# FrozenWolf-Cyber/Indic-CL-ASR

Hardware: AMD Instinct MI355X
Metric: utterances/sec (15 s @16 kHz) Conformer-M RNNT-CTC+EWC train step (higher is better)
Workload: dtype bf16; 1 GPU; BASELINE configs[1]: Conformer-medium (d=256, 16L, H=640) hybrid RNNT-CTC + EWC, bs=32/GPU x 15 s, bf16 projections, freeze_encoder_till=12, 22x257 heads, fused_batch_size=4; global_batch=32, parallelism=dp1

## Files before the change

### include/indicasr.h

```cpp
#ifndef INDICASR_H
#define INDICASR_H

#include <stddef.h>
#include <stdint.h>

#ifdef __cplusplus
extern "C" {
#endif

typedef void* ia_stream_t;

enum ia_status {
    IA_OK = 0,
    IA_INVALID_VALUE = -1,
    IA_WORKSPACE_TOO_SMALL = -2,
    IA_LAUNCH_FAILED = -3,
    IA_UNSUPPORTED = -4,
};

const char* ia_version(void);

size_t ia_rnnt_workspace_bytes(int B, int T, int U1);
int ia_rnnt_loss(const float* logits, const int64_t* labels, const int64_t* act_lens, const int64_t* label_lens,
                 int B, int T, int U1, int V, int blank, float fastemit_lambda, float clamp,
// ... 89 lines not shown
                                int* counts, int* overflow, ia_stream_t stream);
size_t ia_greedy_decode_scratch_bytes(int B, int Hp, int Hj);
int ia_greedy_decode_cluster(int B, int Hp, int Hj);
int ia_greedy_rnnt_decode_bf16w_ex(const float* f_all, const int64_t* out_len, const float* EW, const void* Whh_bf16,
                                   const void* Wpred_bf16, const float* bpred, const void* Whead_bf16, const float* bhead, int B,
                                   int T, int Hp, int Hj, int V, int blank, int row_blank, int row_sos, int max_symbols, int* tokens,
                                   int cap, int* counts, int* overflow, int cluster, void* scratch, size_t scratch_bytes,
                                   ia_stream_t stream);

int ia_edit_distance_batch(const int32_t* a, const int64_t* a_off, const int32_t* b, const int64_t* b_off, int n, int64_t* out);

int ia_quantize_fp8_rows(const void* x, int is_f32, int ld, int64_t M, int K, void* q, int ldq, float* scale, ia_stream_t stream);
int ia_gemm_fp8(const void* Aq, int lda, const float* a_scale, const void* Wq, int ldw, const float* w_scale, int M, int N, int K,
                const float* bias, int act, float dropout_p, unsigned seed, float alpha, const float* R, int ldr, float* outF,
                int ldof, void* outH, int ldoh, ia_stream_t stream);
int ia_subsample_conv1(const float* feats, int B, int Fm, int Tm, int C, const float* w1, const float* b1, void* out,
                       ia_stream_t stream);
int ia_subsample_conv2(const void* in_cl, int B, int T1, int F1, int C, const void* w2r, const float* b2, int N, void* out,
                       ia_stream_t stream);
int ia_gemm_bf16_ln_supported(int N, int K);
int ia_gemm_bf16_ln(const void* A, int lda, const void* W, int ldw, int M, int N, int K, const float* bias, float dropout_p,
                    unsigned seed, float alpha, const float* R, int ldr, float* outF, int ldof, const float* ln_g,
                    const float* ln_b, float ln_eps, void* outH, int ldoh, ia_stream_t stream);
int ia_layernorm(const float* x, int ldx, int N, int d, const float* g1, const float* b1, float eps, float* outF,
                 int ldf, const float* g2, const float* b2, void* outH, int ldh, ia_stream_t stream);
int ia_glu_dwconv(const void* x2, const int64_t* lens, int B, int T, int d, int ksz, const float* w, const float* bias,
                  float* z, float* bn_sum, float* bn_sumsq, float* scratch, ia_stream_t stream);
int64_t ia_dwconv_scratch_elems(int B, int T, int d, int ksz);
int ia_colsum_bf16(const void* x, int M, int N, int ld, float* out, ia_stream_t stream);
int ia_dwconv_time(const float* x, int B, int T, int d, int ksz, const float* w, const float* bias, int flip, float* y,
                   ia_stream_t stream);
int ia_dwconv_time_wgrad(const float* x, const float* dy, int B, int T, int d, int ksz, float* dw, float* db,
                         float* scratch, ia_stream_t stream);
int ia_dwconv_glu_bwd(const float* dz, const void* c2, const int64_t* lens, int B, int T, int d, int ksz, const float* w, void* dc2,
                      ia_stream_t stream);
int ia_dwconv_glu_wgrad(const void* c2, const int64_t* lens, const float* dy, int B, int T, int d, int ksz, float* dw, float* db,
                        float* scratch, ia_stream_t stream);
int ia_bn_silu(const float* z, int64_t n_rows, int d, const float* bn_sum, const float* bn_sumsq, const float* gamma,
               const float* beta, float* running_mean, float* running_var, int64_t* num_batches_tracked,
               float momentum, float eps, int training, void* out, ia_stream_t stream);

int ia_gemm_bnsilu_supported(int K);
int ia_gemm_bnsilu_bf16(const float* z, int ldz, int64_t n_rows, const float* bn_sum, const float* bn_sumsq,
                        const float* gamma, const float* beta, float* running_mean, float* running_var,
                        int64_t* num_batches_tracked, float momentum, float eps, int training, const void* W, int ldw, int M,
                        int N, int K, const float* bias, float dropout_p, unsigned seed, float alpha, const float* R, int ldr,
// ... 230 lines not shown
```

### indic_cl_asr_amd/_lib.py

```python
import ctypes
import os
import subprocess

_HERE = os.path.dirname(os.path.abspath(__file__))
LIB_PATH = os.environ.get("IA_LIB_PATH") or os.path.join(_HERE, "libindicasr_hip.so")

IA_OK = 0
_STATUS = {-1: "IA_INVALID_VALUE", -2: "IA_WORKSPACE_TOO_SMALL", -3: "IA_LAUNCH_FAILED", -4: "IA_UNSUPPORTED"}

_c = ctypes
_vp, _i, _f, _sz = _c.c_void_p, _c.c_int, _c.c_float, _c.c_size_t
_i64 = _c.c_int64

class BlockParams(_c.Structure):
    _fields_ = ([(n, _c.c_void_p) for n in (
        "w_ff1a", "w_ff1b", "w_qkv", "w_pos", "w_out", "w_pw1", "w_pw2", "w_ff2a", "w_ff2b",
        "b_ff1a", "b_ff1b", "b_qkv", "b_out", "b_pw1", "b_pw2", "b_ff2a", "b_ff2b",
        "ln_ff1_g", "ln_ff1_b", "ln_att_g", "ln_att_b", "ln_conv_g", "ln_conv_b", "ln_ff2_g", "ln_ff2_b", "ln_out_g", "ln_out_b",
        "pos_u", "pos_v", "dw_w", "dw_b", "bn_g", "bn_b", "bn_rm", "bn_rv", "bn_nbt")]
        + [(n, _c.c_float) for n in ("ln_eps", "bn_eps", "bn_momentum", "p_drop", "p_ff", "p_att", "fc_factor")]
        + [(n, _c.c_int) for n in ("d", "d_ff", "n_heads", "ksz")]
        + [("pl_cached", _c.c_void_p), ("w_pw1_glu", _c.c_void_p), ("b_pw1_glu", _c.c_void_p)])


# ... 64 lines not shown
    "ia_quantize_mxfp8": (_i, [_vp, _i, _i, _i64, _i, _vp, _i, _vp, _i, _vp]),
    "ia_gemm_mxfp8": (_i, [_vp, _i, _vp, _i, _vp, _i, _vp, _i, _i, _i, _i, _vp, _i, _f, _c.c_uint, _f, _vp, _i, _vp, _i, _vp, _i, _vp]),
    "ia_cast_pad_bf16": (_i, [_vp, _i, _i64, _i, _vp, _i, _vp]),
    "ia_rnnt_lattice": (_i, [_vp, _vp, _i, _i, _i, _f, _i, _vp, _vp, _sz, _vp]),
    "ia_joint_backward_g": (_i, [_vp, _vp, _vp, _vp, _i, _i, _i, _i, _i, _i, _f, _vp, _f, _vp, _i, _i, _vp, _vp, _vp, _sz, _vp, _vp,
                                 _vp]),
    "ia_joint_backward_g_skip": (_i, [_vp, _vp, _vp, _vp, _i, _i, _i, _i, _i, _i, _f, _vp, _f, _vp, _i, _i, _vp, _vp, _vp, _sz, _i, _vp,
                                      _vp, _vp]),
    "ia_joint_backward_g_dbias_scratch_elems": (_i64, [_i]),
    "ia_joint_hidden_t": (_i, [_vp, _vp, _vp, _i, _i, _i, _i, _i, _i, _i, _f, _c.c_uint, _vp]),
    "ia_joint_hidden": (_i, [_vp, _vp, _vp, _i, _i, _i, _i, _i, _f, _c.c_uint, _vp]),
    "ia_joint_dh_reduce": (_i, [_vp, _vp, _vp, _vp, _vp, _vp, _vp, _i, _i, _i, _i, _f, _f, _c.c_uint, _vp, _vp]),
    "ia_joint_dh_reduce_scratch_bytes": (_sz, [_i, _i, _i, _i]),
    "ia_joint_dh_fused_supported": (_i, [_i, _i, _i]),
    "ia_joint_dh_k": (_i, []),
    "ia_joint_dh_fused": (_i, [_vp, _vp, _vp, _vp, _vp, _vp, _vp, _vp, _i, _i, _i, _i, _i, _f, _f, _c.c_uint, _vp, _vp]),
    "ia_joint_dh_fused_ex": (_i, [_vp, _vp, _vp, _vp, _vp, _vp, _vp, _vp, _vp, _vp, _i, _i, _i, _i, _i, _i, _f, _f, _c.c_uint, _vp, _vp]),
    "ia_joint_dh_fused_scratch_bytes": (_sz, [_i, _i, _i, _i]),
    "ia_joint_dw_fused_supported": (_i, [_i, _i, _i]),
    "ia_joint_dw_fused_scratch_elems": (_i64, [_i, _i, _i, _i, _i]),
    "ia_joint_dw_fused": (_i, [_vp, _vp, _vp, _vp, _i, _i, _i, _i, _i, _f, _c.c_uint, _vp, _vp, _vp]),
    "ia_gemm_bf16_ln_supported": (_i, [_i, _i]),
    "ia_gemm_bf16_ln": (_i, [_vp, _i, _vp, _i, _i, _i, _i, _vp, _f, _c.c_uint, _f, _vp, _i, _vp, _i, _vp, _vp, _f, _vp, _i, _vp]),
    "ia_joint_dw_fused_ex": (_i, [_vp, _vp, _vp, _vp, _vp, _i, _i, _i, _i, _i, _f, _c.c_uint, _vp, _vp, _vp]),
    "ia_gemm_bf16": (_i, [_vp, _i, _vp, _i, _i, _i, _i, _vp, _i, _f, _c.c_uint, _f, _vp, _i, _vp, _i, _vp, _i, _vp]),
    "ia_gemm_bf16_ex": (_i, [_vp, _i, _vp, _i, _i, _i, _i, _vp, _i, _f, _c.c_uint, _f, _vp, _i, _vp, _i, _vp, _i, _vp, _i, _vp, _i, _vp]),
    "ia_subsample_conv1": (_i, [_vp, _i, _i, _i, _i, _vp, _vp, _vp, _vp]),
    "ia_subsample_conv2": (_i, [_vp, _i, _i, _i, _i, _vp, _vp, _i, _vp, _vp]),
    "ia_layernorm": (_i, [_vp, _i, _i, _i, _vp, _vp, _f, _vp, _i, _vp, _vp, _vp, _i, _vp]),
    "ia_glu_dwconv": (_i, [_vp, _vp, _i, _i, _i, _i, _vp, _vp, _vp, _vp, _vp, _vp, _vp]),
    "ia_dwconv_scratch_elems": (_i64, [_i, _i, _i, _i]),
    "ia_colsum_bf16": (_i, [_vp, _i, _i, _i, _vp, _vp]),
    "ia_dwconv_time": (_i, [_vp, _i, _i, _i, _i, _vp, _vp, _i, _vp, _vp]),
    "ia_dwconv_time_wgrad": (_i, [_vp, _vp, _i, _i, _i, _i, _vp, _vp, _vp, _vp]),
    "ia_dwconv_glu_bwd": (_i, [_vp, _vp, _vp, _i, _i, _i, _i, _vp, _vp, _vp]),
    "ia_dwconv_glu_wgrad": (_i, [_vp, _vp, _vp, _i, _i, _i, _i, _vp, _vp, _vp, _vp]),
    "ia_bn_silu": (_i, [_vp, _i64, _i, _vp, _vp, _vp, _vp, _vp, _vp, _vp, _f, _f, _i, _vp, _vp]),
    "ia_gemm_bnsilu_supported": (_i, [_i]),
    "ia_gemm_bnsilu_bf16": (_i, [_vp, _i, _i64, _vp, _vp, _vp, _vp, _vp, _vp, _vp, _f, _f, _i, _vp, _i, _i, _i, _i, _vp, _f, _c.c_uint, _f,
                                 _vp, _i, _vp, _i, _vp, _i, _vp, _vp]),
    "ia_gemm_bnsilu_bf16_keep": (_i, [_vp, _i, _i64, _vp, _vp, _vp, _vp, _vp, _vp, _vp, _f, _f, _i, _vp, _i, _i, _i, _i, _vp, _f, _c.c_uint,
                                      _f, _vp, _i, _vp, _i, _vp, _i, _vp, _vp, _i, _vp]),
    "ia_glu_dwconv_fixed": (_i, [_vp, _vp, _i, _i, _i, _i, _vp, _vp, _vp, _vp, _vp]),
    "ia_dwconv_gated_fixed": (_i, [_vp, _vp, _i, _i, _i, _i, _vp, _vp, _vp, _vp, _vp]),
    "ia_attn_vt_elems": (_sz, [_i, _i, _i]),
    "ia_relpos_attention": (_i, [_vp, _vp, _vp, _vp, _vp, _i, _i, _i, _i, _f, _c.c_uint, _vp, _vp, _vp]),
# ... 103 lines not shown
```

### indic_cl_asr_amd/csrc/block_exec.hip

```cpp
#include <hip/hip_runtime.h>

#include <cstdint>
#include <cstdlib>

#include "indicasr.h"
#include "ia_common.h"

namespace {
inline size_t up256(size_t x) { return (x + 255) / 256 * 256; }
constexpr int PREFIX_ACC_LAYERS = 64;

struct PrefixWs {
    size_t y, h, qkv, pl, ctx, c2, z, sums, acc, c3, scr, total;
};

PrefixWs prefix_ws(int B, int T, int d, int d_ff, int ksz, int pos_rows) {
    const size_t N = (size_t)B * T;
    PrefixWs w;
    size_t o = 0;
    w.y = o;    o = up256(o + N * d * 2);
    w.h = o;    o = up256(o + N * d_ff * 2);
    w.qkv = o;  o = up256(o + N * 3 * d * 2);
    w.pl = o;   o = up256(o + (size_t)pos_rows * d * 2);
    w.ctx = o;  o = up256(o + N * d * 2);
// ... 39 lines not shown
    if (seg_begin < 0 || seg_end > 2 * n_layers || seg_begin >= seg_end) return IA_INVALID_VALUE;
    if (!layers || n_layers <= 0 || !x || !pos_emb || !lens || !workspace || B <= 0 || T <= 0) return IA_INVALID_VALUE;
    const ia_block_params& l0 = layers[0];
    const int d = l0.d, d_ff = l0.d_ff, H = l0.n_heads, dk = d / (H > 0 ? H : 1), ksz = l0.ksz;
    if (pos_rows < 2 * T - 1) return IA_INVALID_VALUE;
    const PrefixWs w = prefix_ws(B, T, d, d_ff, ksz, pos_rows);
    if (workspace_bytes < w.total) return IA_WORKSPACE_TOO_SMALL;
    if (H <= 0) return IA_INVALID_VALUE;
    if (!ia_relpos_attention_flash_supported(T, dk)) return IA_UNSUPPORTED;
    char* ws = (char*)workspace;
    void *y = ws + w.y, *h = ws + w.h, *qkv = ws + w.qkv, *pl = ws + w.pl, *ctx = ws + w.ctx, *c2 = ws + w.c2, *c3 = ws + w.c3;
    float *z = (float*)(ws + w.z), *sums = (float*)(ws + w.sums), *scr = (float*)(ws + w.scr);
    long long* acc = (long long*)(ws + w.acc);
    const int N = B * T;
    const char* ffn_env = getenv("IA_PREFIX_FFN");
    const bool ffn_fused = ia_ffn_fused_supported(d, d_ff) != 0 && !(ffn_env && ffn_env[0] == 'g');
    const char* bns_env = getenv("IA_PREFIX_BNSILU");
    const bool bnsilu_fused = ia_gemm_bnsilu_supported(d) != 0 && !(bns_env && bns_env[0] == 's');
    const bool bn_fixed = bnsilu_fused && !bn_synced && seg_begin == 0 && seg_end >= 2 * n_layers && n_layers <= PREFIX_ACC_LAYERS;
    if (bn_fixed && hipMemsetAsync(acc, 0, (size_t)n_layers * IA_BN_ACC_COPIES * 2 * d * sizeof(long long), (hipStream_t)stream) != hipSuccess)
        return IA_LAUNCH_FAILED;
    const char* glu_env = getenv("IA_PREFIX_GLU");
    const bool glu_in_gemm = d % 64 == 0 && !(glu_env && glu_env[0] == 'd');
    if (!ffn_fused && seg_begin == 0)
        IA_TRY(ia_layernorm(x, d, N, d, l0.ln_ff1_g, l0.ln_ff1_b, l0.ln_eps, nullptr, 0, nullptr, nullptr, y, d, stream));
    for (int li = seg_begin / 2; li < n_layers && 2 * li < seg_end; ++li) {
        const ia_block_params& L = layers[li];
        if (L.d != d || L.d_ff != d_ff || L.n_heads != H || L.ksz != ksz) return IA_INVALID_VALUE;
        const unsigned seed = seed_base + seed_stride * (unsigned)li;
        const float p = training ? L.p_drop : 0.f, pff = training ? L.p_ff : 0.f, patt = training ? L.p_att : 0.f;
        const bool first_half = 2 * li >= seg_begin, second_half = 2 * li + 1 < seg_end;
        if (first_half) {
        const char* tail_env = getenv("IA_FFN_TAIL");
        const bool qkv_tail = ffn_fused && !(tail_env && tail_env[0] == '0') && ia_ffn_fused_tail_supported(d, d_ff, 3 * d);
        if (qkv_tail) {
            IA_TRY(ia_ffn_fused_tail(x, N, d, d_ff, L.ln_ff1_g, L.ln_ff1_b, L.ln_eps, L.w_ff1a, L.b_ff1a, L.w_ff1b, L.b_ff1b, L.fc_factor,
                                     pff, seed + 1, p, seed + 2, L.ln_att_g, L.ln_att_b, nullptr, 1, L.w_qkv, L.b_qkv, qkv, 3 * d, stream));
        } else if (ffn_fused) {
            IA_TRY(ia_ffn_fused(x, N, d, d_ff, L.ln_ff1_g, L.ln_ff1_b, L.ln_eps, L.w_ff1a, L.b_ff1a, L.w_ff1b, L.b_ff1b, L.fc_factor,
                                pff, seed + 1, p, seed + 2, L.ln_att_g, L.ln_att_b, y, 1, stream));
        } else {
            IA_TRY(ia_gemm_bf16(y, d, L.w_ff1a, d, N, d_ff, d, L.b_ff1a, 1, pff, seed + 1, 1.f, nullptr, 0, nullptr, 0, h, d_ff, stream));
            IA_TRY(ia_gemm_bf16(h, d_ff, L.w_ff1b, d_ff, N, d, d_ff, L.b_ff1b, 0, p, seed + 2, L.fc_factor, x, d, x, d, nullptr, 0, stream));
        }
        if (!ffn_fused)
            IA_TRY(ia_layernorm(x, d, N, d, L.ln_att_g, L.ln_att_b, L.ln_eps, nullptr, 0, nullptr, nullptr, y, d, stream));
        if (!qkv_tail)
            IA_TRY(ia_gemm_bf16(y, d, L.w_qkv, d, N, 3 * d, d, L.b_qkv, 0, 0.f, 0, 1.f, nullptr, 0, nullptr, 0, qkv, 3 * d, stream));
        const void* plu = L.pl_cached;
        if (!plu) {
            IA_TRY(ia_gemm_bf16(pos_emb, d, L.w_pos, d, pos_rows, d, d, nullptr, 0, 0.f, 0, 1.f, nullptr, 0, nullptr, 0, pl, d, stream));
            plu = pl;
        }
        IA_TRY(ia_relpos_attention_flash(qkv, plu, L.pos_u, L.pos_v, lens, B, T, H, dk, patt, seed + 7, ctx, stream));
        static const bool ln_in_gemm = [] { const char* e = getenv("IA_LN_IN_GEMM"); return !(e && e[0] == '0'); }();
        if (ln_in_gemm && ia_gemm_bf16_ln_supported(d, d)) {
            IA_TRY(ia_gemm_bf16_ln(ctx, d, L.w_out, d, N, d, d, L.b_out, p, seed + 3, 1.f, x, d, x, d, L.ln_conv_g, L.ln_conv_b, L.ln_eps, y, d,
                                   stream));
        } else {
            IA_TRY(ia_gemm_bf16(ctx, d, L.w_out, d, N, d, d, L.b_out, 0, p, seed + 3, 1.f, x, d, x, d, nullptr, 0, stream));
            IA_TRY(ia_layernorm(x, d, N, d, L.ln_conv_g, L.ln_conv_b, L.ln_eps, nullptr, 0, nullptr, nullptr, y, d, stream));
        }
        if (bn_fixed && glu_in_gemm && L.w_pw1_glu && L.b_pw1_glu) {
            IA_TRY(ia_gemm_bf16_ex(y, d, L.w_pw1_glu, d, N, 2 * d, d, L.b_pw1_glu, 4, 0.f, 0, 1.f, nullptr, 0, nullptr, 0, c2, d, nullptr, 0,
                                   nullptr, 0, stream));
            IA_TRY(ia_dwconv_gated_fixed(c2, lens, B, T, d, ksz, L.dw_w, L.dw_b, z, acc + (size_t)li * IA_BN_ACC_COPIES * 2 * d, stream));
        } else {
            IA_TRY(ia_gemm_bf16(y, d, L.w_pw1, d, N, 2 * d, d, L.b_pw1, 0, 0.f, 0, 1.f, nullptr, 0, nullptr, 0, c2, 2 * d, stream));
            if (bn_fixed)
                IA_TRY(ia_glu_dwconv_fixed(c2, lens, B, T, d, ksz, L.dw_w, L.dw_b, z, acc + (size_t)li * IA_BN_ACC_COPIES * 2 * d, stream));
            else
                IA_TRY(ia_glu_dwconv(c2, lens, B, T, d, ksz, L.dw_w, L.dw_b, z, sums, sums + d, scr, stream));
        }
        }
        if (!second_half) break;
        if (bnsilu_fused) {
            IA_TRY(ia_gemm_bnsilu_bf16(z, d, N, sums, sums + d, L.bn_g, L.bn_b, bn_synced ? nullptr : L.bn_rm,
                                       bn_synced ? nullptr : L.bn_rv, bn_synced ? nullptr : L.bn_nbt, L.bn_momentum, L.bn_eps,
                                       training ? 1 : 0, L.w_pw2, d, (int)N, d, d, L.b_pw2, p, seed + 4, 1.f, x, d, x, d, nullptr, 0,
                                       bn_fixed ? acc + (size_t)li * IA_BN_ACC_COPIES * 2 * d : nullptr, stream));
        } else {
            IA_TRY(ia_bn_silu(z, N, d, sums, sums + d, L.bn_g, L.bn_b, bn_synced ? nullptr : L.bn_rm, bn_synced ? nullptr : L.bn_rv,
                              bn_synced ? nullptr : L.bn_nbt, L.bn_momentum, L.bn_eps, training ? 1 : 0, c3, stream));
            IA_TRY(ia_gemm_bf16(c3, d, L.w_pw2, d, N, d, d, L.b_pw2, 0, p, seed + 4, 1.f, x, d, x, d, nullptr, 0, stream));
        }
        if (ffn_fused) {
            IA_TRY(ia_ffn_fused(x, N, d, d_ff, L.ln_ff2_g, L.ln_ff2_b, L.ln_eps, L.w_ff2a, L.b_ff2a, L.w_ff2b, L.b_ff2b, L.fc_factor,
                                pff, seed + 5, p, seed + 6, L.ln_out_g, L.ln_out_b, nullptr, 0, stream));
            continue;
        }
        IA_TRY(ia_layernorm(x, d, N, d, L.ln_ff2_g, L.ln_ff2_b, L.ln_eps, nullptr, 0, nullptr, nullptr, y, d, stream));
        IA_TRY(ia_gemm_bf16(y, d, L.w_ff2a, d, N, d_ff, d, L.b_ff2a, 1, pff, seed + 5, 1.f, nullptr, 0, nullptr, 0, h, d_ff, stream));
        IA_TRY(ia_gemm_bf16(h, d_ff, L.w_ff2b, d_ff, N, d, d_ff, L.b_ff2b, 0, p, seed + 6, L.fc_factor, x, d, x, d, nullptr, 0, stream));
        if (li + 1 < n_layers) {
            const ia_block_params& Nx = layers[li + 1];
// ... 8 lines not shown
```

### indic_cl_asr_amd/csrc/gemm_bf16.hip

```cpp
#include <hip/hip_bf16.h>

#include <stdlib.h>

#include "gemm_common.h"

int ia_gemm_big_wanted(int M, int N, int K, int lda, int ldw, int act);
int ia_gemm_big_launch(const void* gemm_args, hipStream_t st);

namespace {

typedef __bf16 bf8 __attribute__((ext_vector_type(8)));

constexpr int G_BK = 64;
constexpr int G_ROWB = G_BK * 2 + 16;
constexpr int G_THREADS = GEMM_THREADS;
struct ConvRow { int b, t2, f2; };

__device__ __forceinline__ uint4 conv_a_load(const GemmArgs& a, const ConvRow& r, int k0, int kv) {
    const int k = k0 + kv * 8;
    const int tap = k / a.cC, c0 = k - tap * a.cC;
    const int dt = tap / 3, df = tap - dt * 3;
    const int t1 = 2 * r.t2 + dt - 1, f1 = 2 * r.f2 + df - 1;
    if (k >= a.K || r.t2 < 0 || t1 < 0 || t1 >= a.cT1 || f1 < 0 || f1 >= a.cF1) return make_uint4(0, 0, 0, 0);
    return *reinterpret_cast<const uint4*>(a.A + (((size_t)r.b * a.cT1 + t1) * a.cF1 + f1) * a.cC + c0);
}

template <int BM, int BN, bool CONV = false>
__global__ __launch_bounds__(G_THREADS, (BN == 256 ? 2 : (BM == 128 ? 3 : 4))) void gemm_bf16_nt_kernel(GemmArgs a) {
    static_assert(BM == 64 || BM == 96 || BM == 128, "row tiles of 64, 96 or 128");
    constexpr int WM = BM / 2, WN = BN / 2, TI = WM / 16, TJ = WN / 16;
    constexpr int A_BYTES = BM * G_ROWB;
    constexpr int AV = BM * 8 / G_THREADS, BV = BN * 8 / G_THREADS;
    extern __shared__ __attribute__((aligned(16))) unsigned char smem[];
    const int tid = threadIdx.x, lane = tid & 63, wave = tid >> 6;
    const int c = lane & 15, q = lane >> 4;
    const int wm = wave >> 1, wn = wave & 1;
    int m0, n0;
    if (!gemm_xcd_tile<BM, BN>(a.M, a.N, m0, n0)) return;

    static_assert((BV == 4 || BV == 8) && (AV == 2 || AV == 3 || AV == 4), "staging registers are named (arrays end up in scratch)");
    ConvRow crow[4];
    if constexpr (CONV) {
#pragma unroll
        for (int i = 0; i < 4; ++i) {
            const int m = m0 + ((tid + i * G_THREADS) >> 3);
            const int f2 = m % a.cF2, bt = m / a.cF2;
            crow[i].f2 = f2; crow[i].t2 = (m < a.M) ? (bt % a.cT2) : -1; crow[i].b = bt / a.cT2;
        }
    }
    uint4 ra0, ra1, ra2 = make_uint4(0, 0, 0, 0), ra3 = make_uint4(0, 0, 0, 0), rb0, rb1, rb2, rb3;
    uint4 rb4 = make_uint4(0, 0, 0, 0), rb5 = rb4, rb6 = rb4, rb7 = rb4;
#define G_LDK(rowp_, k_) ([&]() { const int kk_ = (k_); const uint4 v_ = *reinterpret_cast<const uint4*>((rowp_) + (kk_ < a.K ? kk_ : 0)); \
                                  return kk_ < a.K ? v_ : make_uint4(0, 0, 0, 0); }())
#define G_LOAD(k0_) \
    do { \
        { const int idx_ = tid + 0 * G_THREADS, kv_ = idx_ & 7; if constexpr (CONV) { ra0 = conv_a_load(a, crow[0], (k0_), kv_); } else { const int row_ = idx_ >> 3; const int gr_ = (m0 + row_ < a.M) ? (m0 + row_) : (a.M - 1); ra0 = G_LDK(a.A + (size_t)gr_ * a.lda, (k0_) + kv_ * 8); } } \
        { const int idx_ = tid + 1 * G_THREADS, kv_ = idx_ & 7; if constexpr (CONV) { ra1 = conv_a_load(a, crow[1], (k0_), kv_); } else { const int row_ = idx_ >> 3; const int gr_ = (m0 + row_ < a.M) ? (m0 + row_) : (a.M - 1); ra1 = G_LDK(a.A + (size_t)gr_ * a.lda, (k0_) + kv_ * 8); } } \
        if constexpr (AV >= 3) { \
        { const int idx_ = tid + 2 * G_THREADS, kv_ = idx_ & 7; if constexpr (CONV) { ra2 = conv_a_load(a, crow[2], (k0_), kv_); } else { const int row_ = idx_ >> 3; const int gr_ = (m0 + row_ < a.M) ? (m0 + row_) : (a.M - 1); ra2 = G_LDK(a.A + (size_t)gr_ * a.lda, (k0_) + kv_ * 8); } } \
        } \
        if constexpr (AV == 4) { \
// ... 14 lines not shown
    do { \
        unsigned char* sa_ = smem; (void)(buf_); \
        unsigned char* sb_ = sa_ + A_BYTES; \
        { const int idx_ = tid + 0 * G_THREADS; *reinterpret_cast<uint4*>(sa_ + (idx_ >> 3) * G_ROWB + (idx_ & 7) * 16) = ra0; } \
        { const int idx_ = tid + 1 * G_THREADS; *reinterpret_cast<uint4*>(sa_ + (idx_ >> 3) * G_ROWB + (idx_ & 7) * 16) = ra1; } \
        if constexpr (AV >= 3) { \
        { const int idx_ = tid + 2 * G_THREADS; *reinterpret_cast<uint4*>(sa_ + (idx_ >> 3) * G_ROWB + (idx_ & 7) * 16) = ra2; } \
        } \
        if constexpr (AV == 4) { \
        { const int idx_ = tid + 3 * G_THREADS; *reinterpret_cast<uint4*>(sa_ + (idx_ >> 3) * G_ROWB + (idx_ & 7) * 16) = ra3; } \
        } \
        { const int idx_ = tid + 0 * G_THREADS; *reinterpret_cast<uint4*>(sb_ + (idx_ >> 3) * G_ROWB + (idx_ & 7) * 16) = rb0; } \
        { const int idx_ = tid + 1 * G_THREADS; *reinterpret_cast<uint4*>(sb_ + (idx_ >> 3) * G_ROWB + (idx_ & 7) * 16) = rb1; } \
        { const int idx_ = tid + 2 * G_THREADS; *reinterpret_cast<uint4*>(sb_ + (idx_ >> 3) * G_ROWB + (idx_ & 7) * 16) = rb2; } \
        { const int idx_ = tid + 3 * G_THREADS; *reinterpret_cast<uint4*>(sb_ + (idx_ >> 3) * G_ROWB + (idx_ & 7) * 16) = rb3; } \
        if constexpr (BV == 8) { \
        { const int idx_ = tid + 4 * G_THREADS; *reinterpret_cast<uint4*>(sb_ + (idx_ >> 3) * G_ROWB + (idx_ & 7) * 16) = rb4; } \
        { const int idx_ = tid + 5 * G_THREADS; *reinterpret_cast<uint4*>(sb_ + (idx_ >> 3) * G_ROWB + (idx_ & 7) * 16) = rb5; } \
        { const int idx_ = tid + 6 * G_THREADS; *reinterpret_cast<uint4*>(sb_ + (idx_ >> 3) * G_ROWB + (idx_ & 7) * 16) = rb6; } \
        { const int idx_ = tid + 7 * G_THREADS; *reinterpret_cast<uint4*>(sb_ + (idx_ >> 3) * G_ROWB + (idx_ & 7) * 16) = rb7; } \
        } \
    } while (0)

    f4 acc[TI][TJ];
#pragma unroll
    for (int i = 0; i < TI; ++i)
#pragma unroll
        for (int j = 0; j < TJ; ++j) acc[i][j] = (f4){0.f, 0.f, 0.f, 0.f};

    const int nk = (a.K + G_BK - 1) / G_BK;
    G_LOAD(0);
    G_STORE(0);
    __syncthreads();
    for (int kt = 0; kt < nk; ++kt) {
        if (kt + 1 < nk) G_LOAD((kt + 1) * G_BK);
        const unsigned char* sa = smem + (wm * WM + c) * G_ROWB + q * 16;
        const unsigned char* sb = smem + A_BYTES + (wn * WN + c) * G_ROWB + q * 16;
#pragma unroll
        for (int ks = 0; ks < G_BK / 32; ++ks) {
            bf8 af[TI], bfr[TJ];
#pragma unroll
            for (int i = 0; i < TI; ++i) af[i] = *reinterpret_cast<const bf8*>(sa + i * 16 * G_ROWB + ks * 64);
#pragma unroll
            for (int j = 0; j < TJ; ++j) bfr[j] = *reinterpret_cast<const bf8*>(sb + j * 16 * G_ROWB + ks * 64);
#pragma unroll
            for (int i = 0; i < TI; ++i)
#pragma unroll
                for (int j = 0; j < TJ; ++j)
                    acc[i][j] = __builtin_amdgcn_mfma_f32_16x16x32_bf16(af[i], bfr[j], acc[i][j], 0, 0, 0);
        }
        __syncthreads();
        if (kt + 1 < nk) {
            G_STORE((kt + 1) & 1);
            __syncthreads();
        }
    }

    gemm_tile_epilogue<BM, BN>(a, acc, smem, m0, n0);
}

constexpr int GD_STAGES = 3;
__device__ __attribute__((aligned(128))) uint4 ia_gemm_zero_page[8];
template <int BM, int BN, bool CONV = false>
__global__ __launch_bounds__(G_THREADS, 2) void gemm_bf16_nt_dma_kernel(GemmArgs a) {
    static_assert(BM == 64 && BN == 128, "issue shares below are written for 64 x 128 tiles");
    constexpr int A_ST = BM * 128, B_ST = BN * 128, STAGE = A_ST + B_ST;
    extern __shared__ __attribute__((aligned(16))) unsigned char smem[];
    const int tid = threadIdx.x, lane = tid & 63;
    const int wave = __builtin_amdgcn_readfirstlane(tid >> 6);
    const int c = lane & 15, q = lane >> 4;
    const int wm = wave >> 1, wn = wave & 1;
    int m0, n0;
    if (!gemm_xcd_tile<BM, BN>(a.M, a.N, m0, n0)) return;

    const int lrow = lane >> 3;
    const unsigned lsw = (unsigned)(((lane & 7) ^ lrow) * 16);
    unsigned aoff[2], boff[4];
    unsigned avalid[2] = {0u, 0u};
#pragma unroll
    for (int i = 0; i < 2; ++i) {
// ... 86 lines not shown
        else asm volatile("s_waitcnt vmcnt(0)" ::: "memory");
        __builtin_amdgcn_s_barrier();
        if (kt + 2 < nk) issue(kt + 2, slot == 0 ? 2 : slot - 1);
        compute(slot);
        slot = slot == 2 ? 0 : slot + 1;
    }
    __syncthreads();
    gemm_tile_epilogue<BM, BN>(a, acc, smem, m0, n0);
}

template <int BM, int BN, bool CONV = false>
int launch_gemm(const GemmArgs& a, hipStream_t st) {
    constexpr int STAGE = (BM + BN) * G_ROWB, EPI = gemm_epi_bytes(BM, BN);
    const size_t lds = STAGE > EPI ? STAGE : EPI;
    const int grid = gemm_xcd_grid(a.M, a.N, BM, BN);
    if (lds > 64 * 1024 &&
        hipFuncSetAttribute((const void*)gemm_bf16_nt_kernel<BM, BN, CONV>, hipFuncAttributeMaxDynamicSharedMemorySize, (int)lds) != hipSuccess)
        return IA_LAUNCH_FAILED;
    hipLaunchKernelGGL((gemm_bf16_nt_kernel<BM, BN, CONV>), dim3(grid), dim3(G_THREADS), lds, st, a);
    IA_RETURN_IF_LAUNCH_FAILED();
    return IA_OK;
}

}

extern "C" int ia_gemm_bf16(const void* A, int lda, const void* W, int ldw, int M, int N, int K, const float* bias,
                            int act, float dropout_p, unsigned seed, float alpha, const float* R, int ldr, float* outF,
                            int ldof, void* outH, int ldoh, ia_stream_t stream) {
    return ia_gemm_bf16_ex(A, lda, W, ldw, M, N, K, bias, act, dropout_p, seed, alpha, R, ldr, outF, ldof, outH, ldoh, nullptr, 0,
                           nullptr, 0, stream);
}

extern "C" int ia_gemm_bf16_ex(const void* A, int lda, const void* W, int ldw, int M, int N, int K, const float* bias,
                               int act, float dropout_p, unsigned seed, float alpha, const float* R, int ldr, float* outF,
                               int ldof, void* outH, int ldoh, void* outPre, int ldpre, const void* aux, int ldaux,
                               ia_stream_t stream) {
    return ia_gemm_bf16_ex2(A, lda, W, ldw, M, N, K, bias, act, dropout_p, seed, alpha, R, ldr, outF, ldof, outH, ldoh, outPre, ldpre, aux,
                            ldaux, 0, stream);
}

extern "C" int ia_gemm_bf16_ex2(const void* A, int lda, const void* W, int ldw, int M, int N, int K, const float* bias,
                                int act, float dropout_p, unsigned seed, float alpha, const float* R, int ldr, float* outF,
                                int ldof, void* outH, int ldoh, void* outPre, int ldpre, const void* aux, int ldaux, int flags,
                                ia_stream_t stream) {
    if (N <= 0 || K <= 0 || (act == 3) != (aux != nullptr)) return IA_INVALID_VALUE;
    const bool unsupported = (outPre && (ldpre % 8 != 0 || !ia_is_aligned(outPre, 16))) || (aux && (ldaux % 8 != 0 || !ia_is_aligned(aux, 16))) ||
// ... 30 lines not shown
            return IA_OK;
        }
    }
    if (best == 128) return launch_gemm<128, 128>(a, st);
    if (best == 96) return launch_gemm<96, 128>(a, st);
    return launch_gemm<64, 128>(a, st);
}

extern "C" int ia_gemm_bf16_ln_supported(int N, int K) { return (N == 256 && K % 8 == 0 && K >= 8) ? 1 : 0; }

extern "C" int ia_gemm_bf16_ln(const void* A, int lda, const void* W, int ldw, int M, int N, int K, const float* bias, float dropout_p,
                               unsigned seed, float alpha, const float* R, int ldr, float* outF, int ldof, const float* ln_g,
                               const float* ln_b, float ln_eps, void* outH, int ldoh, ia_stream_t stream) {
    if (!outF || !outH || !ln_g || !ln_b) return IA_INVALID_VALUE;
    const bool unsupported = !ia_gemm_bf16_ln_supported(N, K) || lda % 8 != 0 || ldw % 8 != 0;
    GemmArgs a = {};
    if (const int rc = gemm_check_and_fill(a, A, W, unsupported, M, N, bias, 0, dropout_p, seed, alpha, R, ldr, outF, ldof, outH, ldoh)) return rc;
    if (!ia_is_aligned(ln_g, 16) || !ia_is_aligned(ln_b, 16)) return IA_INVALID_VALUE;
    a.A = (const __bf16*)A; a.W = (const __bf16*)W; a.K = K; a.lda = lda; a.ldw = ldw;
    a.ln_g = ln_g; a.ln_b = ln_b; a.ln_eps = ln_eps;
    return launch_gemm<64, 256>(a, (hipStream_t)stream);
}

namespace {
__global__ __launch_bounds__(256) void conv1_relu_cl_kernel(const float* __restrict__ x, int B, int Fm, int Tm, int T1, int F1,
                                                            int C, const float* __restrict__ w, const float* __restrict__ bias,
                                                            __bf16* __restrict__ out) {
    const int cg = C / 8;
    const int ppb = 256 / cg;
    if ((int)threadIdx.x >= ppb * cg) return;
    const int c0 = (threadIdx.x % cg) * 8;
    float wr[8][9], br[8];
#pragma unroll
    for (int j = 0; j < 8; ++j) {
        br[j] = bias[c0 + j];
#pragma unroll
        for (int k = 0; k < 9; ++k) wr[j][k] = w[(c0 + j) * 9 + k];
    }
    constexpr int CP1 = 4;
    const int F1g = (F1 + CP1 - 1) / CP1;
    const int64_t ngrp = (int64_t)B * T1 * F1g;
    for (int64_t pg = (int64_t)blockIdx.x * ppb + threadIdx.x / cg; pg < ngrp; pg += (int64_t)gridDim.x * ppb) {
        int64_t q = pg;
        const int fg = (int)(q % F1g); q /= F1g;
        const int t1 = (int)(q % T1);
        const int b = (int)(q / T1);
// ... 67 lines not shown
```

### indic_cl_asr_amd/csrc/gemm_common.h

```cpp
#pragma once
#include <hip/hip_bf16.h>

#include <type_traits>

#include "dropout_mask.h"
#include "ia_common.h"

namespace {

typedef float f4 __attribute__((ext_vector_type(4)));

constexpr int GEMM_THREADS = 256;

struct GemmEpi {
    const float* bias; const float* R;
    float* outF; __bf16* outH;
    int M, N, ldr, ldof, ldoh;
    int act;
    float alpha;
    unsigned seed, thr;
    float keep_scale;
};

struct GemmArgs : GemmEpi {
// ... 80 lines not shown
    const int ntn = (N + BN - 1) / BN;
    const int xcd = blockIdx.x & 7, slot = blockIdx.x >> 3;
    const int mt = xcd + 8 * (slot / ntn);
    m0 = mt * BM; n0 = (slot % ntn) * BN;
    return m0 < M;
}
inline int gemm_xcd_grid(int M, int N, int BM, int BN) {
    const int ntm = (M + BM - 1) / BM, ntn = (N + BN - 1) / BN;
    return 8 * ((ntm + 7) / 8) * ntn;
}

__device__ __forceinline__ float gemm_half_wave_sum(float v) {
    v += IA_DPP_F(0.f, v, 0xB1, 0xF);
    v += IA_DPP_F(0.f, v, 0x4E, 0xF);
    v += IA_DPP_F(0.f, v, 0x141, 0xF);
    v += IA_DPP_F(0.f, v, 0x140, 0xF);
    v += __shfl_xor(v, 16, 64);
    return v;
}

constexpr int gemm_epi_rows(int BM, int BN) { return (BN == 256) ? 32 : ((BM == 96) ? 48 : 64); }
constexpr int gemm_epi_bytes(int BM, int BN) { return gemm_epi_rows(BM, BN) * (BN + 4) * 4; }

template <int BM, int BN, class Args>
__device__ __forceinline__ void gemm_tile_epilogue(const Args& a, f4 (&acc)[BM / 32][BN / 32], unsigned char* smem, int m0, int n0) {
    constexpr bool FULL = std::is_same<Args, GemmArgs>::value;
    constexpr int WM = BM / 2, WN = BN / 2, TI = WM / 16, TJ = WN / 16;
    constexpr int LDC = BN + 4;
    constexpr int EP_ROWS = gemm_epi_rows(BM, BN);
    static_assert(BM % EP_ROWS == 0 && (EP_ROWS % WM == 0 || WM % EP_ROWS == 0), "epilogue passes cover whole wave rows");
    const int tid = threadIdx.x, lane = tid & 63, wave = tid >> 6;
    const int c = lane & 15, q = lane >> 4;
    const int wm = wave >> 1, wn = wave & 1;
    float* sc = reinterpret_cast<float*>(smem);
    constexpr int VEC_PER_ROW = BN / 8;
    for (int pass = 0; pass < BM / EP_ROWS; ++pass) {
    if (pass > 0) __syncthreads();
    if ((wm * WM) / EP_ROWS == pass) {
#pragma unroll
        for (int i = 0; i < TI; ++i)
#pragma unroll
            for (int j = 0; j < TJ; ++j)
#pragma unroll
                for (int r = 0; r < 4; ++r)
                    sc[(wm * WM - pass * EP_ROWS + i * 16 + q * 4 + r) * LDC + wn * WN + j * 16 + c] = acc[i][j][r];
    }
    __syncthreads();
    if constexpr (FULL) {
// ... 25 lines not shown
        if (gm >= a.M || gn >= a.N) continue;
        float v[8];
        const float4 x0 = *reinterpret_cast<const float4*>(sc + row * LDC + cv * 8);
        const float4 x1 = *reinterpret_cast<const float4*>(sc + row * LDC + cv * 8 + 4);
        v[0] = x0.x; v[1] = x0.y; v[2] = x0.z; v[3] = x0.w; v[4] = x1.x; v[5] = x1.y; v[6] = x1.z; v[7] = x1.w;
        gemm_epilogue8(a, gm, gn, v);
        if constexpr (FULL && BN == 256) {
            if (a.ln_g) {
                float s1 = 0.f;
#pragma unroll
                for (int j = 0; j < 8; ++j) s1 += v[j];
                const float mean = gemm_half_wave_sum(s1) * (1.f / 256.f);
                float s2 = 0.f;
#pragma unroll
                for (int j = 0; j < 8; ++j) { v[j] -= mean; s2 += v[j] * v[j]; }
                const float rstd = rsqrtf(gemm_half_wave_sum(s2) * (1.f / 256.f) + a.ln_eps);
                const float4 g0 = *reinterpret_cast<const float4*>(a.ln_g + gn), g1 = *reinterpret_cast<const float4*>(a.ln_g + gn + 4);
                const float4 c0 = *reinterpret_cast<const float4*>(a.ln_b + gn), c1 = *reinterpret_cast<const float4*>(a.ln_b + gn + 4);
                const float gg[8] = {g0.x, g0.y, g0.z, g0.w, g1.x, g1.y, g1.z, g1.w};
                const float bb[8] = {c0.x, c0.y, c0.z, c0.w, c1.x, c1.y, c1.z, c1.w};
                union { uint4 u; __bf16 h[8]; } o;
#pragma unroll
                for (int j = 0; j < 8; ++j) o.h[j] = (__bf16)(v[j] * rstd * gg[j] + bb[j]);
                *reinterpret_cast<uint4*>(a.outH + (size_t)gm * a.ldoh + gn) = o.u;
            }
        }
    }
    }
}

constexpr int GEMM_T_BM = 128, GEMM_T_BN = 128;
constexpr int GEMM_T_EPI = 64 * (GEMM_T_BN + 4) * 4;
template <bool ROW_SCALED, class Args>
__device__ __forceinline__ void gemm_tile_epilogue_t(const Args& a, f4 (&acc)[4][4], unsigned char* smem, int m0, int n0,
                                                     const float* sa = nullptr, const float* sw = nullptr) {
    constexpr int LDC = GEMM_T_BN + 4, VEC_PER_ROW = GEMM_T_BN / 8;
    const int tid = threadIdx.x, lane = tid & 63, wave = tid >> 6;
    const int c = lane & 15, q = lane >> 4;
    const int wm = wave >> 1, wn = wave & 1;
    float* sc = reinterpret_cast<float*>(smem);
    for (int pass = 0; pass < 2; ++pass) {
        if (pass) __syncthreads();
        if (wm == pass) {
#pragma unroll
            for (int i = 0; i < 4; ++i)
#pragma unroll
                for (int j = 0; j < 4; ++j)
// ... 39 lines not shown
```

Before: 3786 utterances/s.

## Fuse out-projection, conv LayerNorm and GLU pointwise GEMM into one kernel

Adds a kernel that runs the attention output projection with residual and LayerNorm, keeps the normalized 64x256 tile in LDS, and immediately multiplies it by the 512-wide GLU pointwise weights. The GLU output is written directly. This drops the bf16 round-trip of the LN output and one kernel launch per layer on the fixed-BN path. In exchange it uses a large-LDS kernel limited to one workgroup per CU, which can cost occupancy and latency hiding compared with the two separate GEMMs.

```diff
diff --git a/include/indicasr.h b/include/indicasr.h
--- a/include/indicasr.h
+++ b/include/indicasr.h
@@ -135,6 +135,11 @@
 int ia_gemm_bf16_ln(const void* A, int lda, const void* W, int ldw, int M, int N, int K, const float* bias, float dropout_p,
                     unsigned seed, float alpha, const float* R, int ldr, float* outF, int ldof, const float* ln_g,
                     const float* ln_b, float ln_eps, void* outH, int ldoh, ia_stream_t stream);
+int ia_gemm_bf16_ln_glu_supported(int N, int K);
+int ia_gemm_bf16_ln_glu(const void* A, int lda, const void* W, int ldw, int M, int N, int K, const float* bias, float dropout_p,
+                        unsigned seed, float alpha, const float* R, int ldr, float* outF, int ldof, const float* ln_g,
+                        const float* ln_b, float ln_eps, const void* W2, int ldw2, const float* bias2, void* outG, int ldog,
+                        ia_stream_t stream);
 int ia_layernorm(const float* x, int ldx, int N, int d, const float* g1, const float* b1, float eps, float* outF,
                  int ldf, const float* g2, const float* b2, void* outH, int ldh, ia_stream_t stream);
 int ia_glu_dwconv(const void* x2, const int64_t* lens, int B, int T, int d, int ksz, const float* w, const float* bias,
diff --git a/indic_cl_asr_amd/_lib.py b/indic_cl_asr_amd/_lib.py
--- a/indic_cl_asr_amd/_lib.py
+++ b/indic_cl_asr_amd/_lib.py
@@ -110,6 +110,9 @@
     "ia_joint_dw_fused": (_i, [_vp, _vp, _vp, _vp, _i, _i, _i, _i, _i, _f, _c.c_uint, _vp, _vp, _vp]),
     "ia_gemm_bf16_ln_supported": (_i, [_i, _i]),
     "ia_gemm_bf16_ln": (_i, [_vp, _i, _vp, _i, _i, _i, _i, _vp, _f, _c.c_uint, _f, _vp, _i, _vp, _i, _vp, _vp, _f, _vp, _i, _vp]),
+    "ia_gemm_bf16_ln_glu_supported": (_i, [_i, _i]),
+    "ia_gemm_bf16_ln_glu": (_i, [_vp, _i, _vp, _i, _i, _i, _i, _vp, _f, _c.c_uint, _f, _vp, _i, _vp, _i, _vp, _vp, _f, _vp, _i, _vp, _vp, _i,
+                                 _vp]),
     "ia_joint_dw_fused_ex": (_i, [_vp, _vp, _vp, _vp, _vp, _i, _i, _i, _i, _i, _f, _c.c_uint, _vp, _vp, _vp]),
     "ia_gemm_bf16": (_i, [_vp, _i, _vp, _i, _i, _i, _i, _vp, _i, _f, _c.c_uint, _f, _vp, _i, _vp, _i, _vp, _i, _vp]),
     "ia_gemm_bf16_ex": (_i, [_vp, _i, _vp, _i, _i, _i, _i, _vp, _i, _f, _c.c_uint, _f, _vp, _i, _vp, _i, _vp, _i, _vp, _i, _vp, _i, _vp]),
diff --git a/indic_cl_asr_amd/csrc/block_exec.hip b/indic_cl_asr_amd/csrc/block_exec.hip
--- a/indic_cl_asr_amd/csrc/block_exec.hip
+++ b/indic_cl_asr_amd/csrc/block_exec.hip
@@ -85,6 +85,12 @@
         return IA_LAUNCH_FAILED;
     const char* glu_env = getenv("IA_PREFIX_GLU");
     const bool glu_in_gemm = d % 64 == 0 && !(glu_env && glu_env[0] == 'd');
+    const char* chain_env = getenv("IA_PREFIX_CHAIN");
+    bool chain_g = true;
+    if (chain_env) {
+        chain_g = false;
+        for (const char* c = chain_env; *c; ++c) chain_g = chain_g || *c == 'g';
+    }
     if (!ffn_fused && seg_begin == 0)
         IA_TRY(ia_layernorm(x, d, N, d, l0.ln_ff1_g, l0.ln_ff1_b, l0.ln_eps, nullptr, 0, nullptr, nullptr, y, d, stream));
     for (int li = seg_begin / 2; li < n_layers && 2 * li < seg_end; ++li) {
@@ -117,6 +123,12 @@
         }
         IA_TRY(ia_relpos_attention_flash(qkv, plu, L.pos_u, L.pos_v, lens, B, T, H, dk, patt, seed + 7, ctx, stream));
         static const bool ln_in_gemm = [] { const char* e = getenv("IA_LN_IN_GEMM"); return !(e && e[0] == '0'); }();
+        const bool glu_fixed = bn_fixed && glu_in_gemm && L.w_pw1_glu && L.b_pw1_glu;
+        if (chain_g && glu_fixed && ln_in_gemm && ia_gemm_bf16_ln_glu_supported(d, d)) {
+            IA_TRY(ia_gemm_bf16_ln_glu(ctx, d, L.w_out, d, N, d, d, L.b_out, p, seed + 3, 1.f, x, d, x, d, L.ln_conv_g, L.ln_conv_b, L.ln_eps,
+                                       L.w_pw1_glu, d, L.b_pw1_glu, c2, d, stream));
+            IA_TRY(ia_dwconv_gated_fixed(c2, lens, B, T, d, ksz, L.dw_w, L.dw_b, z, acc + (size_t)li * IA_BN_ACC_COPIES * 2 * d, stream));
+        } else {
         if (ln_in_gemm && ia_gemm_bf16_ln_supported(d, d)) {
             IA_TRY(ia_gemm_bf16_ln(ctx, d, L.w_out, d, N, d, d, L.b_out, p, seed + 3, 1.f, x, d, x, d, L.ln_conv_g, L.ln_conv_b, L.ln_eps, y, d,
                                    stream));
@@ -124,7 +136,7 @@
             IA_TRY(ia_gemm_bf16(ctx, d, L.w_out, d, N, d, d, L.b_out, 0, p, seed + 3, 1.f, x, d, x, d, nullptr, 0, stream));
             IA_TRY(ia_layernorm(x, d, N, d, L.ln_conv_g, L.ln_conv_b, L.ln_eps, nullptr, 0, nullptr, nullptr, y, d, stream));
         }
-        if (bn_fixed && glu_in_gemm && L.w_pw1_glu && L.b_pw1_glu) {
+        if (glu_fixed) {
             IA_TRY(ia_gemm_bf16_ex(y, d, L.w_pw1_glu, d, N, 2 * d, d, L.b_pw1_glu, 4, 0.f, 0, 1.f, nullptr, 0, nullptr, 0, c2, d, nullptr, 0,
                                    nullptr, 0, stream));
             IA_TRY(ia_dwconv_gated_fixed(c2, lens, B, T, d, ksz, L.dw_w, L.dw_b, z, acc + (size_t)li * IA_BN_ACC_COPIES * 2 * d, stream));
@@ -134,6 +146,7 @@
                 IA_TRY(ia_glu_dwconv_fixed(c2, lens, B, T, d, ksz, L.dw_w, L.dw_b, z, acc + (size_t)li * IA_BN_ACC_COPIES * 2 * d, stream));
             else
                 IA_TRY(ia_glu_dwconv(c2, lens, B, T, d, ksz, L.dw_w, L.dw_b, z, sums, sums + d, scr, stream));
+        }
         }
         }
         if (!second_half) break;
diff --git a/indic_cl_asr_amd/csrc/gemm_bf16.hip b/indic_cl_asr_amd/csrc/gemm_bf16.hip
--- a/indic_cl_asr_amd/csrc/gemm_bf16.hip
+++ b/indic_cl_asr_amd/csrc/gemm_bf16.hip
@@ -25,18 +25,15 @@
     return *reinterpret_cast<const uint4*>(a.A + (((size_t)r.b * a.cT1 + t1) * a.cF1 + f1) * a.cC + c0);
 }
 
-template <int BM, int BN, bool CONV = false>
-__global__ __launch_bounds__(G_THREADS, (BN == 256 ? 2 : (BM == 128 ? 3 : 4))) void gemm_bf16_nt_kernel(GemmArgs a) {
+template <int BM, int BN, bool CONV>
+__device__ __forceinline__ void gemm_bf16_nt_mainloop(const GemmArgs& a, unsigned char* smem, int m0, int n0, f4 (&acc)[BM / 32][BN / 32]) {
     static_assert(BM == 64 || BM == 96 || BM == 128, "row tiles of 64, 96 or 128");
     constexpr int WM = BM / 2, WN = BN / 2, TI = WM / 16, TJ = WN / 16;
     constexpr int A_BYTES = BM * G_ROWB;
     constexpr int AV = BM * 8 / G_THREADS, BV = BN * 8 / G_THREADS;
-    extern __shared__ __attribute__((aligned(16))) unsigned char smem[];
     const int tid = threadIdx.x, lane = tid & 63, wave = tid >> 6;
     const int c = lane & 15, q = lane >> 4;
     const int wm = wave >> 1, wn = wave & 1;
-    int m0, n0;
-    if (!gemm_xcd_tile<BM, BN>(a.M, a.N, m0, n0)) return;
 
     static_assert((BV == 4 || BV == 8) && (AV == 2 || AV == 3 || AV == 4), "staging registers are named (arrays end up in scratch)");
     ConvRow crow[4];
@@ -97,7 +94,6 @@
         } \
     } while (0)
 
-    f4 acc[TI][TJ];
 #pragma unroll
     for (int i = 0; i < TI; ++i)
 #pragma unroll
@@ -130,7 +126,15 @@
             __syncthreads();
         }
     }
-
+}
+
+template <int BM, int BN, bool CONV = false>
+__global__ __launch_bounds__(G_THREADS, (BN == 256 ? 2 : (BM == 128 ? 3 : 4))) void gemm_bf16_nt_kernel(GemmArgs a) {
+    extern __shared__ __attribute__((aligned(16))) unsigned char smem[];
+    int m0, n0;
+    if (!gemm_xcd_tile<BM, BN>(a.M, a.N, m0, n0)) return;
+    f4 acc[BM / 32][BN / 32];
+    gemm_bf16_nt_mainloop<BM, BN, CONV>(a, smem, m0, n0, acc);
     gemm_tile_epilogue<BM, BN>(a, acc, smem, m0, n0);
 }
 
@@ -263,6 +267,72 @@
     return IA_OK;
 }
 
+
+struct GemmLnGluArgs {
+    GemmArgs g;
+    const __bf16* W2;
+    const float* bias2;
+    __bf16* outG;
+    int ldw2, ldog;
+};
+constexpr int LG_STAGE = (64 + 256) * G_ROWB;
+constexpr int LG_A2 = 64 * GEMM_LN_ROWB, LG_W2 = 128 * GEMM_LN_ROWB;
+constexpr int LG_LDS = LG_STAGE + LG_A2 + LG_W2;
+static_assert(gemm_epi_bytes(64, 256) <= LG_STAGE && gemm_epi_bytes(64, 128) <= LG_STAGE, "the epilogue tiles live in the stage");
+static_assert(LG_LDS <= 160 * 1024, "one workgroup's LDS");
+
+__global__ __launch_bounds__(G_THREADS, 1) void gemm_ln_glu_kernel(GemmLnGluArgs p) {
+    extern __shared__ __attribute__((aligned(16))) unsigned char smem[];
+    int m0, n0;
+    if (!gemm_xcd_tile<64, 256>(p.g.M, 256, m0, n0)) return;
+    unsigned char* a2 = smem + LG_STAGE;
+    unsigned char* w2 = a2 + LG_A2;
+    const int tid = threadIdx.x, lane = tid & 63, wave = tid >> 6;
+    const int c = lane & 15, q = lane >> 4;
+    const int wm = wave >> 1, wn = wave & 1;
+
+    f4 acc1[2][8];
+    gemm_bf16_nt_mainloop<64, 256, false>(p.g, smem, m0, n0, acc1);
+
+    uint4 rw0, rw1, rw2, rw3, rw4, rw5, rw6, rw7, rw8, rw9, rw10, rw11, rw12, rw13, rw14, rw15;
+    const __bf16* wsrc = p.W2 + (size_t)(tid >> 5) * p.ldw2 + (tid & 31) * 8;
+    unsigned char* wdst = w2 + (tid >> 5) * GEMM_LN_ROWB + (tid & 31) * 16;
+#define LG_FOR16(X_) X_(0) X_(1) X_(2) X_(3) X_(4) X_(5) X_(6) X_(7) X_(8) X_(9) X_(10) X_(11) X_(12) X_(13) X_(14) X_(15)
+#define LG_ROW(i_) ((i_) * 8)
+#define LG_LOAD(i_) rw##i_ = *reinterpret_cast<const uint4*>(wslab + (size_t)LG_ROW(i_) * p.ldw2);
+#define LG_STORE(i_) *reinterpret_cast<uint4*>(wdst + LG_ROW(i_) * GEMM_LN_ROWB) = rw##i_;
+    { const __bf16* wslab = wsrc; LG_FOR16(LG_LOAD) }
+
+    gemm_tile_epilogue<64, 256>(p.g, acc1, smem, m0, 0, a2);
+
+    GemmArgs e = {};
+    e.bias = p.bias2; e.outH = p.outG; e.M = p.g.M; e.N = 512; e.ldoh = p.ldog; e.act = 4; e.alpha = 1.f; e.keep_scale = 1.f;
+    const unsigned char* sa = a2 + (wm * 32 + c) * GEMM_LN_ROWB + q * 16;
+    const unsigned char* sb = w2 + (wn * 64 + c) * GEMM_LN_ROWB + q * 16;
+    for (int nt = 0; nt < 4; ++nt) {
+        LG_FOR16(LG_STORE)
+        __syncthreads();
+        if (nt + 1 < 4) { const __bf16* wslab = wsrc + (size_t)((nt + 1) * 128) * p.ldw2; LG_FOR16(LG_LOAD) }
+        f4 acc[2][4];
+#pragma unroll
+        for (int i = 0; i < 2; ++i)
+#pragma unroll
+            for (int j = 0; j < 4; ++j) acc[i][j] = (f4){0.f, 0.f, 0.f, 0.f};
+#pragma unroll
+        for (int ks = 0; ks < 256 / 32; ++ks) {
+            bf8 af[2], bfr[4];
+#pragma unroll
+            for (int i = 0; i < 2; ++i) af[i] = *reinterpret_cast<const bf8*>(sa + i * 16 * GEMM_LN_ROWB + ks * 64);
+#pragma unroll
+            for (int j = 0; j < 4; ++j) bfr[j] = *reinterpret_cast<const bf8*>(sb + j * 16 * GEMM_LN_ROWB + ks * 64);
+#pragma unroll
+            for (int i = 0; i < 2; ++i)
+#pragma unroll
+                for (int j = 0; j < 4; ++j) acc[i][j] = __builtin_amdgcn_mfma_f32_16x16x32_bf16(af[i], bfr[j], acc[i][j], 0, 0, 0);
+        }
+        gemm_tile_epilogue<64, 128>(e, acc, smem, m0, nt * 128);
+    }
+}
 }
 
 extern "C" int ia_gemm_bf16(const void* A, int lda, const void* W, int ldw, int M, int N, int K, const float* bias,
@@ -339,6 +409,27 @@
     return launch_gemm<64, 256>(a, (hipStream_t)stream);
 }
 
+extern "C" int ia_gemm_bf16_ln_glu_supported(int N, int K) { return ia_gemm_bf16_ln_supported(N, K); }
+
+extern "C" int ia_gemm_bf16_ln_glu(const void* A, int lda, const void* W, int ldw, int M, int N, int K, const float* bias,
+                                   float dropout_p, unsigned seed, float alpha, const float* R, int ldr, float* outF, int ldof,
+                                   const float* ln_g, const float* ln_b, float ln_eps, const void* W2, int ldw2, const float* bias2,
+                                   void* outG, int ldog, ia_stream_t stream) {
+    if (!outF || !outG || !ln_g || !ln_b || !W2) return IA_INVALID_VALUE;
+    const bool unsupported = !ia_gemm_bf16_ln_glu_supported(N, K) || lda % 8 != 0 || ldw % 8 != 0 || ldw2 % 8 != 0 || ldw2 < N;
+    GemmLnGluArgs p = {};
+    if (const int rc = gemm_check_and_fill(p.g, A, W, unsupported, M, N, bias, 0, dropout_p, seed, alpha, R, ldr, outF, ldof, outG, ldog)) return rc;
+    if (!ia_is_aligned(ln_g, 16) || !ia_is_aligned(ln_b, 16) || !ia_is_aligned(W2, 16) || (bias2 && !ia_is_aligned(bias2, 16)) || ldog < N)
+        return IA_INVALID_VALUE;
+    p.g.A = (const __bf16*)A; p.g.W = (const __bf16*)W; p.g.K = K; p.g.lda = lda; p.g.ldw = ldw;
+    p.g.ln_g = ln_g; p.g.ln_b = ln_b; p.g.ln_eps = ln_eps;
+    p.W2 = (const __bf16*)W2; p.bias2 = bias2; p.outG = (__bf16*)outG; p.ldw2 = ldw2; p.ldog = ldog;
+    IA_SET_MAX_LDS_ONCE(gemm_ln_glu_kernel, LG_LDS);
+    hipLaunchKernelGGL(gemm_ln_glu_kernel, dim3(gemm_xcd_grid(M, N, 64, 256)), dim3(G_THREADS), LG_LDS, (hipStream_t)stream, p);
+    IA_RETURN_IF_LAUNCH_FAILED();
+    return IA_OK;
+}
+
 namespace {
 __global__ __launch_bounds__(256) void conv1_relu_cl_kernel(const float* __restrict__ x, int B, int Fm, int Tm, int T1, int F1,
                                                             int C, const float* __restrict__ w, const float* __restrict__ bias,
diff --git a/indic_cl_asr_amd/csrc/gemm_common.h b/indic_cl_asr_amd/csrc/gemm_common.h
--- a/indic_cl_asr_amd/csrc/gemm_common.h
+++ b/indic_cl_asr_amd/csrc/gemm_common.h
@@ -126,8 +126,10 @@
 constexpr int gemm_epi_rows(int BM, int BN) { return (BN == 256) ? 32 : ((BM == 96) ? 48 : 64); }
 constexpr int gemm_epi_bytes(int BM, int BN) { return gemm_epi_rows(BM, BN) * (BN + 4) * 4; }
 
+constexpr int GEMM_LN_ROWB = 256 * 2 + 16;
 template <int BM, int BN, class Args>
-__device__ __forceinline__ void gemm_tile_epilogue(const Args& a, f4 (&acc)[BM / 32][BN / 32], unsigned char* smem, int m0, int n0) {
+__device__ __forceinline__ void gemm_tile_epilogue(const Args& a, f4 (&acc)[BM / 32][BN / 32], unsigned char* smem, int m0, int n0,
+                                                   unsigned char* ln_rows = nullptr) {
     constexpr bool FULL = std::is_same<Args, GemmArgs>::value;
     constexpr int WM = BM / 2, WN = BN / 2, TI = WM / 16, TJ = WN / 16;
     constexpr int LDC = BN + 4;
@@ -199,7 +201,8 @@
                 union { uint4 u; __bf16 h[8]; } o;
 #pragma unroll
                 for (int j = 0; j < 8; ++j) o.h[j] = (__bf16)(v[j] * rstd * gg[j] + bb[j]);
-                *reinterpret_cast<uint4*>(a.outH + (size_t)gm * a.ldoh + gn) = o.u;
+                if (ln_rows) *reinterpret_cast<uint4*>(ln_rows + (pass * EP_ROWS + row) * GEMM_LN_ROWB + cv * 16) = o.u;
+                else *reinterpret_cast<uint4*>(a.outH + (size_t)gm * a.ldoh + gn) = o.u;
             }
         }
     }
```

Measured after the change: 3779 utterances/s. No clear change (-0.2%).
